# crowsonkb/style_transfer2

Measured on AMD Instinct MI355X. Metric: style-transfer iters/sec @1024px VGG19, higher is better.
Workload: dtype f32; 1 GPU; configs[1]: 1024x1024 single image per GPU, VGG19 to conv5_1, content conv4_2 + 5 style layers, adam fp32, 500 iterations per image; jobs=1, parallelism=independent jobs, 1 per GPU, no collective (replicas)

## Files before the change

style_transfer2_amd/csrc/conv3x3_winograd.hip:

```cpp
#include <hip/hip_runtime.h>
#include <stdint.h>
#include <stdlib.h>
#include <string.h>
#include <type_traits>
#include "st2_kernels.h"
#include "env.h"

namespace st2 {

typedef float f32x16 __attribute__((ext_vector_type(16)));
typedef float f32x4 __attribute__((ext_vector_type(4)));


constexpr int WN_CH = 8;
constexpr int WN_IW = 40;
constexpr int WN_V = 4 * 16 * 64;

size_t wino_pack_floats(int K, int M) { return (size_t)((M + 127) / 128 * 4) * (K / 2) * 1024; }

static void wino_pack(const float* w, int Cout, int Cin, bool dgrad, float* dst)
{
    const int K = dgrad ? Cout : Cin, M = dgrad ? Cin : Cout, nkp = K / 2;
    memset(dst, 0, wino_pack_floats(K, M) * sizeof(float));
    static const double G[4][3] = {{1, 0, 0}, {0.5, 0.5, 0.5}, {0.5, -0.5, 0.5}, {0, 0, 1}};
    for (int m = 0; m < M; ++m)
        for (int k = 0; k < K; ++k) {
            double g[3][3], t[4][3], u[4][4];
            for (int tap = 0; tap < 9; ++tap)
                g[tap / 3][tap % 3] = dgrad ? w[((size_t)k * Cin + m) * 9 + (8 - tap)] : w[((size_t)m * Cin + k) * 9 + tap];
            for (int i = 0; i < 4; ++i)
                for (int j = 0; j < 3; ++j) t[i][j] = G[i][0] * g[0][j] + G[i][1] * g[1][j] + G[i][2] * g[2][j];
            for (int i = 0; i < 4; ++i)
                for (int j = 0; j < 4; ++j) u[i][j] = t[i][0] * G[j][0] + t[i][1] * G[j][1] + t[i][2] * G[j][2];
            const size_t base = ((size_t)(m / 32) * nkp + k / 2) * 1024;
            const int lane = (k & 1) * 32 + (m & 31);
            for (int pos = 0; pos < 16; ++pos)
                dst[base + ((size_t)(pos >> 2) * 64 + lane) * 4 + (pos & 3)] = (float)u[pos >> 2][pos & 3];
        }
}
void pack_wino_weights_fwd(const float* w, int Cout, int Cin, float* dst) { wino_pack(w, Cout, Cin, false, dst); }
void pack_wino_weights_dgrad(const float* w, int Cout, int Cin, float* dst) { wino_pack(w, Cout, Cin, true, dst); }

struct WinoKArgs {
    const float* in; const float4* upack; const float* bias; float* out;
    const float* mask_src; const float* inject;
    int K, M, H, W, nch, tiles_x, tiles_y, n_mtiles, relu;
    unsigned in_bytes, u_bytes;
    float* pool_out; int pool_h, pool_w;
    unsigned char* pool_amap;
    const unsigned char* unpool_amap; unsigned amap_bytes; int ph, pw;
    int splits; float* scratch;
    unsigned long long* stamps;
};

typedef __attribute__((address_space(3))) void* lptr_t;
constexpr unsigned kOOB = 0xffffffffu;

__device__ __forceinline__ float f4c(const float4& v, int i) { return i == 0 ? v.x : i == 1 ? v.y : i == 2 ? v.z : v.w; }

template <int EPI, bool RS> struct WinoEpiOps {
    static constexpr bool E_FWD = EPI == 1 || EPI == 2, E_MASK = EPI == 3;
    static constexpr int NEB = RS ? 2 : 4;
    static constexpr int NG = E_MASK ? 2 * NEB : NEB;
    static constexpr int UNDER = NG < 4 ? NG : 4;
    int mw, dm0, odd;
    bool live, has_inj;
    unsigned row0, plane4, out_bytes;
    float mk[E_MASK ? NEB : 1][E_MASK ? 4 : 1][4], ij[E_FWD ? 1 : NEB][E_FWD ? 1 : 4][4], bs[E_FWD ? NEB : 1][E_FWD ? 4 : 1];

    __device__ __forceinline__ void init(const WinoKArgs& a, int lane, int yw, int x0, int m0, int ph, unsigned plane)
    {
        odd = lane & 1;
        const int gy = yw + 2 * ((lane & 31) >> 4) + odd;
        const int gx4 = x0 + 2 * (lane & 14);
        live = gx4 < a.W && gy < a.H;
        mw = m0 + 4 * (lane >> 5);
        dm0 = RS ? 16 * ph : 0;
        has_inj = a.inject != nullptr;
        plane4 = plane * 4u;
        out_bytes = (unsigned)a.M * plane4;
        row0 = ((unsigned)mw * plane + (live ? (unsigned)gy * a.W + gx4 : 0u)) * 4u;
    }
    __device__ __forceinline__ unsigned row_off(const WinoKArgs& a, int ebl, int ee) const
    {
        const int dm = dm0 + 8 * ebl + ee;
        return (live & (mw + dm < a.M)) ? row0 + (unsigned)dm * plane4 : kOOB;
    }
    __device__ __forceinline__ void load(const WinoKArgs& a, int g)
    {
        const int ebl = E_MASK ? g >> 1 : g;
        const bool mask = E_MASK && (g & 1) == 0;
        const __amdgpu_buffer_rsrc_t rs = E_FWD ? __builtin_amdgcn_make_buffer_rsrc((void*)a.bias, 0, (unsigned)a.M * 4u, 0x00020000)
                                        : mask ? __builtin_amdgcn_make_buffer_rsrc((void*)a.mask_src, 0, out_bytes, 0x00020000)
                                               : __builtin_amdgcn_make_buffer_rsrc((void*)a.inject, 0, has_inj ? out_bytes : 0u, 0x00020000);
#pragma unroll
        for (int ee = 0; ee < 4; ++ee) {
            if constexpr (E_FWD) {
                bs[ebl][ee] = __builtin_bit_cast(float, __builtin_amdgcn_raw_buffer_load_b32(rs, (mw + dm0 + 8 * ebl + ee) * 4, 0, 0));
            } else {
                const uint4 v = __builtin_bit_cast(uint4, __builtin_amdgcn_raw_buffer_load_b128(rs, row_off(a, ebl, ee), 0, 0));
                float (&d4)[4] = mask ? mk[E_MASK ? ebl : 0][E_MASK ? ee : 0] : ij[ebl][ee];
                d4[0] = __builtin_bit_cast(float, v.x); d4[1] = __builtin_bit_cast(float, v.y); d4[2] = __builtin_bit_cast(float, v.z); d4[3] = __builtin_bit_cast(float, v.w);
            }
        }
        asm volatile("" ::: "memory");
    }
};
template <bool RS> struct WinoEpiOps<0, RS> {};

template <int WM, int TG, int DIAG = 0, bool QUAD = true, bool PS = false, bool W8 = false, bool H4 = false, bool UNPOOL = false, bool BIG = false,
          bool NOOUT = false, int EPI = 0>
__device__ __forceinline__ void conv3x3_wino_body(const WinoKArgs& a)
{
    static_assert(EPI == 0 || (QUAD && TG == 1 && !PS && !W8 && !BIG && DIAG == 0), "specialised epilogues: aligned widths, one tile group, four waves, below 4 GiB");
    static_assert(!NOOUT || EPI == 0 || EPI == 2, "no-output builds pool");
    static_assert(!NOOUT || (QUAD && TG == 1 && !PS && !W8 && !UNPOOL && !BIG && DIAG == 0), "no-output builds: the builds that write the arg-max map");
    static_assert(!BIG || (QUAD && TG == 1 && !PS && !W8 && DIAG == 0), "big tensors: aligned widths, one tile group, four waves");
    static_assert(!UNPOOL || (QUAD && TG == 1 && !PS && !W8), "unpool: aligned widths, one tile group, four waves");
    static_assert(H4 || (WM * TG == 4 && (TG == 1 || TG == 2)), "4 waves");
    static_assert(!PS || (WM == 2 && TG == 2), "position split: 2 channel slices x 2 position halves");
    static_assert(!W8 || (WM == 4 && TG == 1 && QUAD && !PS), "eight waves: 4 channel slices x 2 position halves, aligned widths");
    static_assert(!H4 || (WM == 2 && TG == 1 && QUAD && !PS && !W8), "half tile: 2 channel slices x 2 position halves, aligned widths");
    constexpr bool RS = W8 || H4;
    constexpr bool AMAP = QUAD && TG == 1;
    constexpr int NW = W8 ? 8 : 4;
    constexpr int PARTNER = W8 ? 4 : 2;
    constexpr bool SPLIT = PS || RS;
    constexpr int BM = 32 * WM;
    constexpr int PROWS = 4 * TG;
    constexpr int IN_ROWS = PROWS + 2;
    constexpr int IW = QUAD ? WN_IW : 64;
    constexpr int COL0 = QUAD ? 3 : 0;
    constexpr int PLANE = IN_ROWS * IW;
    constexpr int UP_ROWS = PROWS / 2 + 2, UP_COLS = 24;
    constexpr int UP_PLANE = UP_ROWS * UP_COLS;
    constexpr int UP_F = WN_CH * UP_PLANE;
    constexpr int UP_FQ = UP_F / 256, UP_AQ = UP_F / 256;
    static_assert(!UNPOOL || (UP_F % 256 == 0 && NW == 4), "unpool staging is a whole number of wave-DMAs");
    constexpr int N_RAW = UNPOOL ? UP_F + UP_F / 4 : WN_CH * PLANE;
    constexpr int I_PER_WAVE = UNPOOL ? (UP_FQ + UP_AQ + NW - 1) / NW
                             : QUAD ? (N_RAW / 4 + 64 * NW - 1) / (64 * NW) : WN_CH * IN_ROWS / 4;
    constexpr int RAW = UNPOOL ? 1024 : QUAD ? I_PER_WAVE * NW * 256 : N_RAW;
    static_assert(QUAD || (WN_CH * IN_ROWS) % 4 == 0, "rows divide over the four waves");

    __shared__ __attribute__((aligned(16))) float raw_s[2][RAW];
    __shared__ __attribute__((aligned(16))) float v_s[2][TG][WN_V];
    __shared__ __attribute__((aligned(16))) float x8_own[W8 ? 8 * 8 * 64 * 4 : 4];
    static_assert(!H4 || 4 * 8 * 64 * 4 <= 2 * TG * WN_V, "H4: the exchange buffer fits the V images");
    float* const x8_s = H4 ? &v_s[0][0][0] : x8_own;

    const int tid = threadIdx.x;
    const int lane = tid & 63;
    const int wave = __builtin_amdgcn_readfirstlane(tid >> 6);
    const int wave_m = W8 ? (wave & 3) : H4 ? (wave & 1) : wave / TG, wave_g = RS ? 0 : wave % TG;
    const int ph = W8 ? wave >> 2 : H4 ? wave >> 1 : wave_g;

    const int nwg = gridDim.x / a.splits;
    const int split = blockIdx.x / nwg, orig = blockIdx.x - split * nwg;
    const int nch = a.nch / a.splits, c_first = split * nch;
    const int xcd = orig & 7, q = nwg >> 3, r = nwg & 7;
    const int logical = (xcd < r ? xcd * (q + 1) : r * (q + 1) + (xcd - r) * q) + (orig >> 3);
    const int n_pt = a.tiles_x * a.tiles_y;
    const int mt = logical / n_pt;
    const int pt = logical - mt * n_pt;
    const int tx = pt % a.tiles_x;
    const int ty = pt / a.tiles_x;
    const int y0 = ty * PROWS, x0 = tx * 32;
    const unsigned plane = (unsigned)a.H * a.W;
    const int nkp = a.K >> 1;

    const unsigned long long t_begin = DIAG ? __builtin_amdgcn_s_memtime() : 0ull;

    const __amdgpu_buffer_rsrc_t rs_i = __builtin_amdgcn_make_buffer_rsrc((void*)a.in, 0, a.in_bytes, 0x00020000);
    const __amdgpu_buffer_rsrc_t rs_a = __builtin_amdgcn_make_buffer_rsrc((void*)(UNPOOL ? a.unpool_amap : nullptr), 0, UNPOOL ? a.amap_bytes : 0u, 0x00020000);
    const unsigned pplane = UNPOOL ? (unsigned)a.ph * a.pw : 0u;
    unsigned ioff[QUAD ? I_PER_WAVE : 1];
    if (UNPOOL) {
#pragma unroll
        for (int t = 0; t < I_PER_WAVE; ++t) {
            const int piece = wave + NW * t;
            const bool bytes = piece >= UP_FQ;
            const int e = ((bytes ? piece - UP_FQ : piece) * 64 + lane) * 4;
            const int c = e / UP_PLANE;
            const int rem = e - c * UP_PLANE;
            const int rr = rem / UP_COLS;
            const int col = rem - rr * UP_COLS;
            const int gy = (y0 >> 1) - 1 + rr, gx = (x0 >> 1) - 4 + col;
            const bool ok = piece < UP_FQ + UP_AQ && gy >= 0 && gy < a.ph && gx >= 0 && gx + 3 < a.pw;
            ioff[t] = ok ? ((unsigned)((BIG && !bytes ? 0 : c_first * WN_CH) + c) * pplane + (unsigned)gy * a.pw + gx) * (bytes ? 1u : 4u) : kOOB;
        }
    } else if (QUAD) {
#pragma unroll
        for (int t = 0; t < I_PER_WAVE; ++t) {
            const int e = ((wave + NW * t) * 64 + lane) * 4;
            const int c = e / PLANE;
            const int rem = e - c * PLANE;
            const int rr = rem / IW;
            const int col = rem - rr * IW;
            const int gy = y0 - 1 + rr, gx = x0 - 4 + col;
            const bool ok = e < N_RAW && gy >= 0 && gy < a.H && gx >= 0 && gx + 3 < a.W;
            ioff[t] = ok ? ((unsigned)((BIG ? 0 : c_first * WN_CH) + c) * plane + (unsigned)gy * a.W + gx) * 4u : kOOB;
        }
    } else {
        const int gx = x0 - 1 + lane;
        ioff[0] = (lane < 34 && gx >= 0 && gx < a.W) ? (unsigned)gx * 4u : kOOB;
    }
    auto dma_raw = [&](int ch, int buf) {
        const __amdgpu_buffer_rsrc_t rs_c = BIG ? __builtin_amdgcn_make_buffer_rsrc(
            (void*)(a.in + (size_t)(c_first + ch) * WN_CH * (UNPOOL ? pplane : plane)), 0, a.in_bytes, 0x00020000) : rs_i;
        if (UNPOOL) {
#pragma unroll
            for (int t = 0; t < I_PER_WAVE; ++t) {
                const int piece = wave + NW * t;
                if (piece < UP_FQ) {
                    const unsigned vo = (ioff[t] == kOOB || BIG) ? ioff[t] : ioff[t] + (unsigned)ch * WN_CH * pplane * 4u;
                    __builtin_amdgcn_raw_ptr_buffer_load_lds(rs_c, (lptr_t)(raw_s[buf] + piece * 256), 16, vo, 0, 0, 0);
                } else if (piece < UP_FQ + UP_AQ) {
                    const unsigned vo = ioff[t] == kOOB ? kOOB : ioff[t] + (unsigned)ch * WN_CH * pplane;
                    __builtin_amdgcn_raw_ptr_buffer_load_lds(rs_a, (lptr_t)(raw_s[buf] + UP_F + (piece - UP_FQ) * 64), 4, vo, 0, 0, 0);
                }
            }
        } else if (QUAD) {
            const unsigned coff = BIG ? 0u : (unsigned)ch * WN_CH * plane * 4u;
#pragma unroll
            for (int t = 0; t < I_PER_WAVE; ++t) {
                const unsigned vo = ioff[t] == kOOB ? kOOB : ioff[t] + coff;
                __builtin_amdgcn_raw_ptr_buffer_load_lds(rs_c, (lptr_t)(raw_s[buf] + (wave + NW * t) * 256), 16, vo, 0, 0, 0);
            }
        } else {
#pragma unroll
            for (int t = 0; t < I_PER_WAVE; ++t) {
                const int row = wave + 4 * t;
                const int c = row / IN_ROWS, gy = y0 - 1 + (row - c * IN_ROWS);
                const bool row_ok = gy >= 0 && gy < a.H;
                const unsigned base = ((unsigned)((c_first + ch) * WN_CH + c) * plane + (unsigned)(row_ok ? gy : 0) * a.W) * 4u;
                const unsigned vo = (row_ok && ioff[0] != kOOB) ? ioff[0] + base : kOOB;
                __builtin_amdgcn_raw_ptr_buffer_load_lds(rs_i, (lptr_t)(raw_s[buf] + row * 64), 4, vo, 0, 0, 0);
            }
        }
    };

    const int xt = tid & 31, xch = (tid >> 5) & 7;
    const int x_raw = UNPOOL ? xch * UP_PLANE + (xt >> 4) * UP_COLS + (xt & 15) + 3
                             : xch * PLANE + (2 * (xt >> 4)) * IW + 2 * (xt & 15) + COL0;
    const int x_v = (((xch >> 1) * 4) * 64 + (xch & 1) * 32 + xt) * 4;
    float d[TG][16];
    auto pin = [&]() {
#pragma unroll
        for (int g = 0; g < TG; ++g) {
            asm volatile("" : "+v"(d[g][0]), "+v"(d[g][1]), "+v"(d[g][2]), "+v"(d[g][3]), "+v"(d[g][4]), "+v"(d[g][5]), "+v"(d[g][6]), "+v"(d[g][7]));
            asm volatile("" : "+v"(d[g][8]), "+v"(d[g][9]), "+v"(d[g][10]), "+v"(d[g][11]), "+v"(d[g][12]), "+v"(d[g][13]), "+v"(d[g][14]), "+v"(d[g][15]));
        }
    };
    float up_v[UNPOOL ? 9 : 1];
    unsigned up_m[UNPOOL ? 9 : 1];
    auto up_expand = [&]() {
        if constexpr (UNPOOL) {
#pragma unroll
            for (int i = 0; i < 4; ++i)
#pragma unroll
                for (int j = 0; j < 4; ++j) {
                    const int r = (i + 1) >> 1, cc = (j + 1) >> 1;
                    const unsigned want = 4u | (2u * ((i + 1) & 1)) | ((j + 1) & 1);
                    d[0][4 * i + j] = up_m[3 * r + cc] == want ? up_v[3 * r + cc] : 0.f;
                }
        }
    };
    auto xf_read = [&](const float* rp) {
        if constexpr (UNPOOL) {
            const unsigned char* bp = reinterpret_cast<const unsigned char*>(rp - x_raw + UP_F) + x_raw;
#pragma unroll
            for (int r = 0; r < 3; ++r)
#pragma unroll
                for (int cc = 0; cc < 3; ++cc) {
                    up_v[3 * r + cc] = rp[r * UP_COLS + cc];
                    up_m[3 * r + cc] = bp[r * UP_COLS + cc];
                }
            return;
        }
#pragma unroll
        for (int g = 0; g < TG; ++g)
#pragma unroll
            for (int i = 0; i < 4; ++i)
#pragma unroll
                for (int j = 0; j < 4; ++j) d[g][4 * i + j] = rp[(4 * g + i) * IW + j];
    };
    auto xf_math = [&]() {
#pragma unroll
        for (int g = 0; g < TG; ++g) {
            float wv[16];
#pragma unroll
            for (int j = 0; j < 4; ++j) {
                wv[j] = d[g][j] - d[g][8 + j]; wv[4 + j] = d[g][4 + j] + d[g][8 + j];
                wv[8 + j] = d[g][8 + j] - d[g][4 + j]; wv[12 + j] = d[g][4 + j] - d[g][12 + j];
            }
#pragma unroll
            for (int i = 0; i < 4; ++i) {
                d[g][4 * i] = wv[4 * i] - wv[4 * i + 2]; d[g][4 * i + 1] = wv[4 * i + 1] + wv[4 * i + 2];
                d[g][4 * i + 2] = wv[4 * i + 2] - wv[4 * i + 1]; d[g][4 * i + 3] = wv[4 * i + 1] - wv[4 * i + 3];
            }
        }
    };
    auto xf_write = [&](float* vp) {
#pragma unroll
        for (int g = 0; g < TG; ++g)
#pragma unroll
            for (int i = 0; i < 4; ++i)
                *reinterpret_cast<float4*>(vp + g * WN_V + i * 256) = make_float4(d[g][4 * i], d[g][4 * i + 1], d[g][4 * i + 2], d[g][4 * i + 3]);
    };

    const f32x4* up = reinterpret_cast<const f32x4*>(a.upack) + ((size_t)(mt * WM + wave_m) * nkp + 4 * c_first) * 256 + lane;
    constexpr int UQ = SPLIT ? 2 : 4;
    f32x4 ua[4][UQ];
    auto u_fill = [&](int kp) {
#pragma unroll
        for (int g = 0; g < UQ; ++g) ua[kp & 3][g] = up[((size_t)kp * 4 + (SPLIT ? 2 * ph + g : g)) * 64];
        asm volatile("" ::: "memory");
    };
    auto u_pin = [&](int set) {
        if constexpr (SPLIT) asm volatile("" : "+v"(ua[set][0]), "+v"(ua[set][1]));
        else asm volatile("" : "+v"(ua[set][0]), "+v"(ua[set][1]), "+v"(ua[set][2]), "+v"(ua[set][3]));
    };
    constexpr int NACC = RS ? 8 : 16;
    constexpr int NBQ = NACC / 4;
    f32x4 bq[2][NBQ];
    auto b_fetch = [&](int buf, int kpl, int set) {
#pragma unroll
        for (int pg = 0; pg < NBQ; ++pg) {
            const float* vimg = PS ? v_s[buf][pg >> 1] : v_s[buf][wave_g];
            const int quad = PS ? 2 * ph + (pg & 1) : (RS ? 2 * ph + pg : pg);
            bq[set][pg] = *reinterpret_cast<const f32x4*>(vimg + ((kpl * 4 + quad) * 64 + lane) * 4);
        }
    };
    auto b_pin = [&](int set) {
        if constexpr (RS) asm volatile("" : "+v"(bq[set][1]));
        else asm volatile("" : "+v"(bq[set][1]), "+v"(bq[set][2]), "+v"(bq[set][3]));
    };

    f32x16 acc[NACC];
#pragma unroll
    for (int p = 0; p < NACC; ++p)
#pragma unroll
        for (int e = 0; e < 16; ++e) acc[p][e] = 0.f;

    dma_raw(0, 0);
    if (nch > 1) dma_raw(1, 1);
    u_fill(0); u_fill(1); u_fill(2);
    __syncthreads();
    if (!W8 || ph == 0) {
        xf_read(raw_s[0] + x_raw);
        up_expand();
        xf_math();
        xf_write(&v_s[0][0][0] + x_v);
    }
    __syncthreads();
    b_fetch(0, 0, 0);

    unsigned long long t0 = 0, r0 = 0;
    if (DIAG) { t0 = __builtin_amdgcn_s_memtime(); r0 = __builtin_amdgcn_s_memrealtime(); }

    WinoEpiOps<EPI, RS> eo;
    if constexpr (EPI != 0) eo.init(a, lane, y0 + 4 * wave_g, x0, mt * BM + wave_m * 32, ph, plane);

    auto chunk = [&](const int c, auto more_t, auto more2_t) {
        constexpr bool MORE = decltype(more_t)::value, MORE2 = decltype(more2_t)::value;
        const int cur = c & 1;
        const bool do_xf = !W8 || ph == ((c + 1) & 1);
#pragma unroll
        for (int kpl = 0; kpl < 4; ++kpl) {
            const int kp = 4 * c + kpl;
            const int set = kpl & 1;
#pragma unroll
            for (int p = 0; p < NACC; ++p) {
                acc[p] = __builtin_amdgcn_mfma_f32_32x32x2f32(ua[kpl][SPLIT ? (p >> 2) & 1 : p >> 2][p & 3], bq[set][p >> 2][p & 3], acc[p], 0, 0, 0);
                if (p == 0) {
                    __builtin_amdgcn_sched_barrier(0);
                    b_pin(set);
                    if (kpl < 3) b_fetch(cur, kpl + 1, set ^ 1);
                    else if (MORE) {
                        if constexpr (SPLIT) asm volatile("s_waitcnt vmcnt(4) lgkmcnt(0)\n\ts_barrier" ::: "memory");
                        else asm volatile("s_waitcnt vmcnt(8) lgkmcnt(0)\n\ts_barrier" ::: "memory");
                        b_fetch(cur ^ 1, 0, 0);
                    }
                    if (MORE || kpl == 0) u_fill(kp + 3);
                    if constexpr (EPI != 0) {
                        if constexpr (!MORE) {
                            constexpr int UNDER = WinoEpiOps<EPI, RS>::UNDER;
                            if (kpl >= 4 - UNDER) eo.load(a, kpl - (4 - UNDER));
                        }
                    }
                    if (MORE && do_xf) {
                        if (kpl == 0) xf_read(raw_s[cur ^ 1] + x_raw);
                        if (kpl == 1) { up_expand(); pin(); xf_math(); pin(); }
                        if (kpl == 2) xf_write(&v_s[cur ^ 1][0][0] + x_v);
                    }
                    if (MORE2 && kpl == 0) dma_raw(c + 2, cur);
                    if (MORE || kpl < 3) u_pin((kpl + 1) & 3);
                    __builtin_amdgcn_sched_barrier(0);
                }
            }
            __builtin_amdgcn_sched_barrier(0);
        }
    };
    {
        using T = std::true_type; using F = std::false_type;
        int c = 0;
        for (; c + 2 < nch; ++c) chunk(c, T{}, T{});
        if (c + 1 < nch) { chunk(c, T{}, F{}); ++c; }
        chunk(c, F{}, F{});
    }
    if constexpr (EPI != 0) {
        if constexpr (!RS && EPI == 2) {
#pragma unroll
            for (int p = 0; p < NACC; ++p) asm volatile("" : "+a"(acc[p]));
        }
#pragma unroll
        for (int g = WinoEpiOps<EPI, RS>::UNDER; g < WinoEpiOps<EPI, RS>::NG; ++g) eo.load(a, g);
        asm volatile("" : "+v"(eo.row0));
        __builtin_amdgcn_sched_barrier(0);
    }

    unsigned long long t_loop_end = 0;
    if (DIAG) {
        const unsigned long long t1 = __builtin_amdgcn_s_memtime(), r1 = __builtin_amdgcn_s_memrealtime();
        t_loop_end = t1;
        if (tid == 0 && a.stamps) { a.stamps[2 * blockIdx.x] = t1 - t0; a.stamps[2 * blockIdx.x + 1] = r1 - r0; }
    }
    float* const xbuf = &v_s[0][0][0];
    auto partial_out = [&](auto grp_t, auto e0_t, int el, float (&y)[4]) {
        constexpr int grp = decltype(grp_t)::value, e0 = decltype(e0_t)::value;
        float t0[4], t1[4];
#pragma unroll
        for (int j = 0; j < 4; ++j) {
            const float ra = acc[(grp * 8 + j) % NACC][e0 + el], rb = acc[(grp * 8 + 4 + j) % NACC][e0 + el];
            if (ph == 0) { t0[j] = ra + rb; t1[j] = rb; }
            else { t0[j] = ra; t1[j] = -ra - rb; }
        }
        y[0] = t0[0] + t0[1] + t0[2]; y[1] = t0[1] - t0[2] - t0[3];
        y[2] = t1[0] + t1[1] + t1[2]; y[3] = t1[1] - t1[2] - t1[3];
    };
    if constexpr (PS) {
        __syncthreads();
#pragma unroll
        for (int e = 0; e < 16; ++e) {
            float y[4];
            if (wave_g == 0) partial_out(std::integral_constant<int, 1>{}, std::integral_constant<int, 0>{}, e, y);
            else partial_out(std::integral_constant<int, 0>{}, std::integral_constant<int, 0>{}, e, y);
            *reinterpret_cast<float4*>(xbuf + ((wave * 16 + e) * 64 + lane) * 4) = make_float4(y[0], y[1], y[2], y[3]);
        }
        __syncthreads();
    }
    if constexpr (RS) {
        if constexpr (H4) __syncthreads();
#pragma unroll
        for (int el = 0; el < 8; ++el) {
            float y[4];
            if (ph == 0) partial_out(std::integral_constant<int, 0>{}, std::integral_constant<int, 8>{}, el, y);
            else partial_out(std::integral_constant<int, 0>{}, std::integral_constant<int, 0>{}, el, y);
            *reinterpret_cast<float4*>(x8_s + ((wave * 8 + el) * 64 + lane) * 4) = make_float4(y[0], y[1], y[2], y[3]);
        }
        __syncthreads();
    }
    auto out_xf = [&](int e, float& y00, float& y01, float& y10, float& y11) {
        if constexpr (RS) {
            float y[4];
            if (ph == 0) partial_out(std::integral_constant<int, 0>{}, std::integral_constant<int, 0>{}, e, y);
            else partial_out(std::integral_constant<int, 0>{}, std::integral_constant<int, 8>{}, e, y);
            const float4 o = *reinterpret_cast<const float4*>(x8_s + (((wave ^ PARTNER) * 8 + e) * 64 + lane) * 4);
            y00 = y[0] + o.x; y01 = y[1] + o.y; y10 = y[2] + o.z; y11 = y[3] + o.w;
        } else if constexpr (PS) {
            float y[4];
            if (wave_g == 0) partial_out(std::integral_constant<int, 0>{}, std::integral_constant<int, 0>{}, e, y);
            else partial_out(std::integral_constant<int, 1>{}, std::integral_constant<int, 0>{}, e, y);
            const float4 o = *reinterpret_cast<const float4*>(xbuf + (((wave ^ 1) * 16 + e) * 64 + lane) * 4);
            y00 = y[0] + o.x; y01 = y[1] + o.y; y10 = y[2] + o.z; y11 = y[3] + o.w;
        } else {
            float tt[2][4];
#pragma unroll
            for (int j = 0; j < 4; ++j) {
                tt[0][j] = acc[j][e] + acc[4 + j][e] + acc[(8 + j) % NACC][e];
                tt[1][j] = acc[4 + j][e] - acc[(8 + j) % NACC][e] - acc[(12 + j) % NACC][e];
            }
            y00 = tt[0][0] + tt[0][1] + tt[0][2]; y01 = tt[0][1] - tt[0][2] - tt[0][3];
            y10 = tt[1][0] + tt[1][1] + tt[1][2]; y11 = tt[1][1] - tt[1][2] - tt[1][3];
        }
    };
  if (!QUAD) {
    const int t31 = lane & 31, khalf = lane >> 5;
    const int gy0 = y0 + 4 * wave_g + 2 * (t31 >> 4), gx = x0 + 2 * (t31 & 15);
    const bool part = a.splits > 1;
    const bool has_bias = !part && a.bias != nullptr, has_mask = !part && a.mask_src != nullptr, has_inj = !part && a.inject != nullptr;
    const bool relu = !part && a.relu;
    float* const outp = part ? a.scratch + (size_t)split * a.M * plane : a.out;
    const bool live = gx < a.W && gy0 < a.H;
    const bool row1 = gy0 + 1 < a.H, col1 = gx + 1 < a.W, wide = (a.W & 1) == 0;
    const int mw = mt * BM + wave_m * 32 + 4 * khalf;
    const unsigned pix0 = live ? (unsigned)gy0 * a.W + gx : 0u, pix1 = (live && row1) ? pix0 + a.W : pix0;
    auto ld2 = [&](const float* base, unsigned off) -> float2 {
        if (wide) return *reinterpret_cast<const float2*>(base + off);
        return make_float2(base[off], col1 ? base[off + 1] : 0.f);
    };
#pragma unroll
    for (int eb = 0; eb < 4; ++eb) {
        const int mb = mw + 8 * eb;
        unsigned off[4];
        float2 mk[4][2], ij[4][2];
        float bs[4];
#pragma unroll
        for (int ee = 0; ee < 4; ++ee) {
            const int m = mb + ee < a.M ? mb + ee : a.M - 1;
            off[ee] = (unsigned)m * plane;
            bs[ee] = has_bias ? a.bias[m] : 0.f;
        }
        if (has_mask) {
#pragma unroll
            for (int ee = 0; ee < 4; ++ee) { mk[ee][0] = ld2(a.mask_src, off[ee] + pix0); mk[ee][1] = ld2(a.mask_src, off[ee] + pix1); }
        }
        if (has_inj) {
#pragma unroll
            for (int ee = 0; ee < 4; ++ee) { ij[ee][0] = ld2(a.inject, off[ee] + pix0); ij[ee][1] = ld2(a.inject, off[ee] + pix1); }
        }
#pragma unroll
        for (int ee = 0; ee < 4; ++ee) {
            const int e = 4 * eb + ee;
            float o[2][2];
            out_xf(e, o[0][0], o[0][1], o[1][0], o[1][1]);
            if (a.pool_out && live && mb + ee < a.M) {
                float pm = o[0][0];
                if (col1) pm = pm > o[0][1] ? pm : o[0][1];
                if (row1) { pm = pm > o[1][0] ? pm : o[1][0]; if (col1) pm = pm > o[1][1] ? pm : o[1][1]; }
                pm += bs[ee];
                if (relu) pm = pm > 0.f ? pm : 0.f;
                a.pool_out[((size_t)(mb + ee) * a.pool_h + (gy0 >> 1)) * a.pool_w + (gx >> 1)] = pm;
            }
#pragma unroll
            for (int i = 0; i < 2; ++i) {
                float o0 = o[i][0] + bs[ee], o1 = o[i][1] + bs[ee];
                if (relu) { o0 = o0 > 0.f ? o0 : 0.f; o1 = o1 > 0.f ? o1 : 0.f; }
                if (has_mask) { o0 = mk[ee][i].x > 0.f ? o0 : 0.f; o1 = mk[ee][i].y > 0.f ? o1 : 0.f; }
                if (has_inj) { o0 += ij[ee][i].x; o1 += ij[ee][i].y; }
                if (live && mb + ee < a.M && (i == 0 || row1)) {
                    float* dst = outp + off[ee] + (i ? pix1 : pix0);
                    if (wide) *reinterpret_cast<float2*>(dst) = make_float2(o0, o1);
                    else { dst[0] = o0; if (col1) dst[1] = o1; }
                }
            }
        }
    }
  } else if constexpr (EPI != 0) {
    constexpr bool E_FWD = EPI == 1 || EPI == 2, E_POOL = EPI == 2, E_MASK = EPI == 3;
    constexpr int NEB = RS ? 2 : 4;
    typedef unsigned wn_u32x4 __attribute__((ext_vector_type(4)));
    const int t31 = lane & 31;
    const __amdgpu_buffer_rsrc_t rs_o = __builtin_amdgcn_make_buffer_rsrc((void*)a.out, 0, NOOUT ? 0u : eo.out_bytes, 0x00020000);
    const int ty2 = y0 + 4 * wave_g + 2 * (t31 >> 4), tx2 = x0 + 2 * (t31 & 15);
    const bool plive = E_POOL && tx2 < a.W && ty2 < a.H, prow1 = ty2 + 1 < a.H;
    const unsigned pplane = E_POOL ? (unsigned)a.pool_h * a.pool_w : 0u;
    const unsigned ppix = plive ? (unsigned)(ty2 >> 1) * a.pool_w + (tx2 >> 1) : 0u;
    const __amdgpu_buffer_rsrc_t rs_po = __builtin_amdgcn_make_buffer_rsrc((void*)a.pool_out, 0, E_POOL ? (unsigned)a.M * pplane * 4u : 0u, 0x00020000);
    const __amdgpu_buffer_rsrc_t rs_pa = __builtin_amdgcn_make_buffer_rsrc((void*)a.pool_amap, 0, (E_POOL && a.pool_amap) ? (unsigned)a.M * pplane : 0u, 0x00020000);
#pragma unroll
    for (int ebl = 0; ebl < NEB; ++ebl) {
        const int mb = eo.mw + eo.dm0 + 8 * ebl;
        if constexpr (!RS && !E_POOL) {
#pragma unroll
            for (int p = 0; p < NACC; ++p) asm volatile("" : "+a"(acc[p]));
        }
#pragma unroll
        for (int ee = 0; ee < 4; ++ee) {
            const int e = 4 * ebl + ee;
            float y00, y01, y10, y11;
            out_xf(e, y00, y01, y10, y11);
            if constexpr (E_POOL) {
                const float b = eo.bs[E_FWD ? ebl : 0][E_FWD ? ee : 0];
                float pm = y00 > y01 ? y00 : y01;
                const float p1 = y10 > y11 ? y10 : y11, pm2 = pm > p1 ? pm : p1;
                pm = prow1 ? pm2 : pm;
                const float qb = pm + b;
                const unsigned slot = y00 + b == qb ? 0u : (y01 + b == qb ? 1u : (y10 + b == qb ? 2u : 3u));
                const unsigned po = (plive && mb + ee < a.M) ? (unsigned)(mb + ee) * pplane + ppix : kOOB;
                __builtin_amdgcn_raw_buffer_store_b8((unsigned char)(slot | (qb > 0.f ? 4u : 0u)), rs_pa, po, 0, 0);
                pm += b;
                pm = pm > 0.f ? pm : 0.f;
                __builtin_amdgcn_raw_buffer_store_b32(__builtin_bit_cast(unsigned, pm), rs_po, po == kOOB ? kOOB : po * 4u, 0, 0);
            }
            if constexpr (NOOUT) continue;
            const float s0 = eo.odd ? y00 : y10, s1 = eo.odd ? y01 : y11;
            const float r0 = __builtin_bit_cast(float, __builtin_amdgcn_update_dpp(0, __builtin_bit_cast(int, s0), 0xB1, 0xf, 0xf, true));
            const float r1 = __builtin_bit_cast(float, __builtin_amdgcn_update_dpp(0, __builtin_bit_cast(int, s1), 0xB1, 0xf, 0xf, true));
            float o[4];
            o[0] = eo.odd ? r0 : y00; o[1] = eo.odd ? r1 : y01; o[2] = eo.odd ? y10 : r0; o[3] = eo.odd ? y11 : r1;
#pragma unroll
            for (int j = 0; j < 4; ++j) {
                if constexpr (E_FWD) {
                    o[j] += eo.bs[E_FWD ? ebl : 0][E_FWD ? ee : 0];
                    o[j] = o[j] > 0.f ? o[j] : 0.f;
                } else {
                    if constexpr (E_MASK) o[j] = eo.mk[E_MASK ? ebl : 0][E_MASK ? ee : 0][j] > 0.f ? o[j] : 0.f;
                    const float oi = o[j] + eo.ij[E_FWD ? 0 : ebl][E_FWD ? 0 : ee][j];
                    o[j] = eo.has_inj ? oi : o[j];
                }
            }
            wn_u32x4 ov;
#pragma unroll
            for (int j = 0; j < 4; ++j) ov[j] = __builtin_bit_cast(unsigned, o[j]);
            __builtin_amdgcn_raw_buffer_store_b128(ov, rs_o, eo.row_off(a, ebl, ee), 0, 0);
        }
        __builtin_amdgcn_sched_barrier(0);
    }
  } else {
    const int t31 = lane & 31, khalf = lane >> 5;
    const int odd = lane & 1;
    const int gy = y0 + 4 * wave_g + 2 * (t31 >> 4) + odd;
    const int gx4 = x0 + 2 * (t31 & 14);
    const bool part = a.splits > 1;
    const bool has_bias = !part && a.bias != nullptr, has_mask = !part && a.mask_src != nullptr, has_inj = !part && a.inject != nullptr;
    const bool relu = !part && a.relu;
    float* const outp = part ? a.scratch + (size_t)split * a.M * plane : a.out;
    const bool live = gx4 < a.W && gy < a.H;
// ... 292 lines not shown
```

style_transfer2_amd/csrc/gram.hip:

```cpp
#include "st2_kernels.h"
#include "env.h"
#include "wave_reduce.h"
#include <stdint.h>
#include <stdlib.h>

namespace st2 {

typedef float f32x16 __attribute__((ext_vector_type(16)));

constexpr int GKT = 32;
constexpr int GLD = GKT + 1;

GramPlan gram_plan(int C, int hw)
{
    GramPlan p;
    p.bt = C > 64 ? 128 : 64;
    const int t = (C + p.bt - 1) / p.bt;
    p.tiles = t * (t + 1) / 2;
    const int target128 = (int)env_int("ST2_GRAM_BLOCKS", 512), target64 = (int)env_int("ST2_GRAM_BLOCKS64", 1024);
    int want = p.bt == 128 ? target128 / p.tiles : (target64 + p.tiles - 1) / p.tiles;
    const int max_splits = (hw + 4 * GKT - 1) / (4 * GKT);
    if (want > max_splits) want = max_splits;
    if (want < 1) want = 1;
    int kslab = (hw + want - 1) / want;
    kslab = (kslab + GKT - 1) / GKT * GKT;
    p.kslab = kslab;
    p.splits = (hw + kslab - 1) / kslab;
    p.slab_floats = (size_t)p.splits * C * C;
    return p;
}

GramPlan gram_plan16(int C, int hw)
{
    GramPlan p = gram_plan(C, hw);
    p.kslab = (p.kslab + 63) / 64 * 64;
    p.splits = (hw + p.kslab - 1) / p.kslab;
    p.slab_floats = (size_t)p.splits * C * C;
    return p;
}

template <int BT>
__global__ __launch_bounds__(256) void gram_partial_k(const float* __restrict__ F, float* __restrict__ slabs,
                                                      int C, int hw, int tiles_1d, int kslab, GramRoi roi)
{
    constexpr int T = BT / 64;
    constexpr int ROWS_PER_T = BT / 8;
    __shared__ float As[BT * GLD];
    __shared__ float Bs[BT * GLD];

    const int tid = threadIdx.x, lane = tid & 63, wave = tid >> 6;
    const int wm = wave >> 1, wn = wave & 1;
    const int n_ut = tiles_1d * (tiles_1d + 1) / 2;
    int tile = blockIdx.x % n_ut;
    const int split = blockIdx.x / n_ut;
    int ti = 0;
    while (tile >= tiles_1d - ti) { tile -= tiles_1d - ti; ++ti; }
    const int tj = ti + tile;
    const int i0 = ti * BT, j0 = tj * BT;
    const bool diag = ti == tj;
    const int kbeg = split * kslab;
    const int kend = min(hw, kbeg + kslab);

    const int sk = tid & 31, sr = tid >> 5;
    float ra[ROWS_PER_T], rb[ROWS_PER_T];

    auto load = [&](int k0) {
        const int k = k0 + sk;
        const int ky = k / roi.rw, kx = k - ky * roi.rw;
        const size_t pix = (size_t)(roi.y0 + ky) * roi.pitch + roi.x0 + kx;
#pragma unroll
        for (int it = 0; it < ROWS_PER_T; ++it) {
            const int r = sr + it * 8;
            ra[it] = (i0 + r < C && k < kend) ? F[(size_t)(i0 + r) * roi.plane + pix] : 0.f;
            if (!diag) rb[it] = (j0 + r < C && k < kend) ? F[(size_t)(j0 + r) * roi.plane + pix] : 0.f;
        }
    };
    auto store = [&]() {
#pragma unroll
        for (int it = 0; it < ROWS_PER_T; ++it) {
            const int r = sr + it * 8;
            As[r * GLD + sk] = ra[it];
            if (!diag) Bs[r * GLD + sk] = rb[it];
        }
    };

    f32x16 acc[T][T];
#pragma unroll
    for (int i = 0; i < T; ++i)
#pragma unroll
        for (int j = 0; j < T; ++j)
#pragma unroll
            for (int e = 0; e < 16; ++e) acc[i][j][e] = 0.f;

    const float* bsrc = diag ? As : Bs;
    const int khalf = lane >> 5, l31 = lane & 31;
    const float* a_base = As + (wm * (T * 32) + l31) * GLD + khalf;
    const float* b_base = bsrc + (wn * (T * 32) + l31) * GLD + khalf;

    load(kbeg);
    for (int k0 = kbeg; k0 < kend; k0 += GKT) {
        __syncthreads();
        store();
        __syncthreads();
        if (k0 + GKT < kend) load(k0 + GKT);
#pragma unroll
        for (int ks = 0; ks < GKT / 2; ++ks) {
            float av[T], bv[T];
#pragma unroll
            for (int i = 0; i < T; ++i) av[i] = a_base[i * 32 * GLD + 2 * ks];
#pragma unroll
            for (int j = 0; j < T; ++j) bv[j] = b_base[j * 32 * GLD + 2 * ks];
#pragma unroll
            for (int i = 0; i < T; ++i)
#pragma unroll
                for (int j = 0; j < T; ++j)
                    acc[i][j] = __builtin_amdgcn_mfma_f32_32x32x2f32(av[i], bv[j], acc[i][j], 0, 0, 0);
        }
    }

    float* dst = slabs + (size_t)split * C * C;
#pragma unroll
    for (int i = 0; i < T; ++i)
#pragma unroll
        for (int j = 0; j < T; ++j) {
            const int col = j0 + wn * (T * 32) + j * 32 + l31;
#pragma unroll
            for (int e = 0; e < 16; ++e) {
                const int row = i0 + wm * (T * 32) + i * 32 + (e & 3) + 8 * (e >> 2) + 4 * khalf;
                if (row < C && col < C) dst[(size_t)row * C + col] = acc[i][j][e];
            }
        }
}

typedef __attribute__((address_space(3))) void* gram_lptr_t;
typedef float gf32x4 __attribute__((ext_vector_type(4)));

template <int BT>
__device__ __forceinline__ void gram_partial_dma_body(const float* __restrict__ F, unsigned f_bytes, float* __restrict__ slabs,
                                                      int C, int hw, int tiles_1d, int kslab)
{
    constexpr int T = BT / 64;
    constexpr int IMG = BT * 32;
    constexpr int PIECES = IMG / 256;
    constexpr int PPW = PIECES / 4;
    __shared__ __attribute__((aligned(16))) float smem[2][2][IMG];

    const int tid = threadIdx.x, lane = tid & 63;
    const int wave = __builtin_amdgcn_readfirstlane(tid >> 6);
    const int wm = wave >> 1, wn = wave & 1;
    const int n_ut = tiles_1d * (tiles_1d + 1) / 2;
    int tile = blockIdx.x % n_ut;
    const int split = blockIdx.x / n_ut;
    int ti = 0;
    while (tile >= tiles_1d - ti) { tile -= tiles_1d - ti; ++ti; }
    const int tj = ti + tile;
    const int i0 = ti * BT, j0 = tj * BT;
    const bool diag = ti == tj;
    const int kbeg = split * kslab;
    const int kend = min(hw, kbeg + kslab);
    const int nsteps = (kend - kbeg) / 32;

    const __amdgpu_buffer_rsrc_t rs = __builtin_amdgcn_make_buffer_rsrc((void*)F, 0, f_bytes, 0x00020000);
    unsigned aoff[PPW], boff[PPW];
#pragma unroll
    for (int t = 0; t < PPW; ++t) {
        const int slot = (wave + 4 * t) * 64 + lane;
        const int r = slot >> 3, q = (slot & 7) ^ ((r >> 1) & 7);
        aoff[t] = i0 + r < C ? ((unsigned)(i0 + r) * (unsigned)hw + (unsigned)kbeg + 4u * q) * 4u : 0xffffffffu;
        boff[t] = j0 + r < C ? ((unsigned)(j0 + r) * (unsigned)hw + (unsigned)kbeg + 4u * q) * 4u : 0xffffffffu;
    }
    auto dma = [&](int step, int stage) {
        const unsigned so = (unsigned)step * 128u;
#pragma unroll
        for (int t = 0; t < PPW; ++t) {
            __builtin_amdgcn_raw_ptr_buffer_load_lds(rs, (gram_lptr_t)(smem[stage][0] + (wave + 4 * t) * 256), 16,
                                                     aoff[t] == 0xffffffffu ? aoff[t] : aoff[t] + so, 0, 0, 0);
            if (!diag)
                __builtin_amdgcn_raw_ptr_buffer_load_lds(rs, (gram_lptr_t)(smem[stage][1] + (wave + 4 * t) * 256), 16,
                                                         boff[t] == 0xffffffffu ? boff[t] : boff[t] + so, 0, 0, 0);
        }
    };

    f32x16 acc[T][T];
#pragma unroll
    for (int i = 0; i < T; ++i)
#pragma unroll
        for (int j = 0; j < T; ++j)
#pragma unroll
            for (int e = 0; e < 16; ++e) acc[i][j][e] = 0.f;

    const int l31 = lane & 31;
    const bool hi = lane >= 32;
    int arow[T], brow[T];
#pragma unroll
    for (int i = 0; i < T; ++i) { arow[i] = wm * (T * 32) + i * 32 + l31; brow[i] = wn * (T * 32) + i * 32 + l31; }

    if (nsteps > 0) dma(0, 0);
    for (int st = 0; st < nsteps; ++st) {
        const int cur = st & 1;
        asm volatile("s_waitcnt vmcnt(0)" ::: "memory");
        __syncthreads();
        if (st + 1 < nsteps) dma(st + 1, cur ^ 1);
        const float* As = smem[cur][0];
        const float* Bs = diag ? smem[cur][0] : smem[cur][1];
#pragma unroll
        for (int q = 0; q < 8; ++q) {
            float a0[T], a1[T], b0[T], b1[T];
#pragma unroll
            for (int i = 0; i < T; ++i) {
                const gf32x4 v = *reinterpret_cast<const gf32x4*>(As + (arow[i] * 8 + (q ^ ((arow[i] >> 1) & 7))) * 4);
                a0[i] = hi ? v.y : v.x; a1[i] = hi ? v.w : v.z;
            }
#pragma unroll
            for (int j = 0; j < T; ++j) {
                const gf32x4 v = *reinterpret_cast<const gf32x4*>(Bs + (brow[j] * 8 + (q ^ ((brow[j] >> 1) & 7))) * 4);
                b0[j] = hi ? v.y : v.x; b1[j] = hi ? v.w : v.z;
            }
#pragma unroll
            for (int i = 0; i < T; ++i)
#pragma unroll
                for (int j = 0; j < T; ++j) {
                    acc[i][j] = __builtin_amdgcn_mfma_f32_32x32x2f32(a0[i], b0[j], acc[i][j], 0, 0, 0);
                    acc[i][j] = __builtin_amdgcn_mfma_f32_32x32x2f32(a1[i], b1[j], acc[i][j], 0, 0, 0);
                }
        }
    }

    const int khalf = lane >> 5;
    float* dst = slabs + (size_t)split * C * C;
#pragma unroll
    for (int i = 0; i < T; ++i)
#pragma unroll
        for (int j = 0; j < T; ++j) {
            const int col = j0 + wn * (T * 32) + j * 32 + l31;
#pragma unroll
            for (int e = 0; e < 16; ++e) {
                const int row = i0 + wm * (T * 32) + i * 32 + (e & 3) + 8 * (e >> 2) + 4 * khalf;
                if (row < C && col < C) dst[(size_t)row * C + col] = acc[i][j][e];
            }
        }
}

__global__ __launch_bounds__(256, 2) void gram_partial_dma_128(const float* F, unsigned f_bytes, float* slabs, int C, int hw, int tiles_1d, int kslab)
{ gram_partial_dma_body<128>(F, f_bytes, slabs, C, hw, tiles_1d, kslab); }
__global__ __launch_bounds__(256, 2) void gram_partial_dma_64(const float* F, unsigned f_bytes, float* slabs, int C, int hw, int tiles_1d, int kslab)
{ gram_partial_dma_body<64>(F, f_bytes, slabs, C, hw, tiles_1d, kslab); }

hipError_t launch_gram_partial(const float* F, float* slabs, int C, int hw, const GramPlan& pl, hipStream_t s,
                               const GramRoi* roi_in)
{
    const int t1 = (C + pl.bt - 1) / pl.bt;
    const unsigned grid = (unsigned)(pl.tiles * pl.splits);
    GramRoi roi = roi_in ? *roi_in : GramRoi{0, 0, hw, hw, (size_t)hw};
    if (!roi_in && !env_off("ST2_GRAM_DMA") && hw % 32 == 0 && pl.kslab % 32 == 0 && (reinterpret_cast<uintptr_t>(F) & 15) == 0 &&
        4ull * C * hw < 0xfffffff0ull) {
        const unsigned fb = (unsigned)(4ull * C * hw);
        if (pl.bt == 128) gram_partial_dma_128<<<grid, 256, 0, s>>>(F, fb, slabs, C, hw, t1, pl.kslab);
        else gram_partial_dma_64<<<grid, 256, 0, s>>>(F, fb, slabs, C, hw, t1, pl.kslab);
        return hipGetLastError();
    }
    if (pl.bt == 128) gram_partial_k<128><<<grid, 256, 0, s>>>(F, slabs, C, hw, t1, pl.kslab, roi);
    else gram_partial_k<64><<<grid, 256, 0, s>>>(F, slabs, C, hw, t1, pl.kslab, roi);
    return hipGetLastError();
}

__global__ __launch_bounds__(256) void gram_reduce_k(const float* __restrict__ slabs, const float* __restrict__ target,
                                                     float* __restrict__ out, float* __restrict__ partial,
                                                     int cc, int splits, float n, int C, int out_ld, int bt)
{
    __shared__ float scratch[4];
    float acc[1] = {0.f};
    for (int i = blockIdx.x * 256 + threadIdx.x; i < cc; i += gridDim.x * 256) {
        const int r = i / C, c = i - r * C;
        const int tr = r / bt, tc = c / bt;
        if (tr > tc) continue;
        float sum = 0.f;
        for (int s = 0; s < splits; ++s) sum += slabs[(size_t)s * cc + i];
        float v = sum / n;
        if (target) v -= target[i];
        out[r * out_ld + c] = v;
        acc[0] += v * v;
        if (tr < tc) { out[c * out_ld + r] = v; acc[0] += v * v; }
    }
    block_sum(acc, scratch);
    if (threadIdx.x == 0 && partial) partial[blockIdx.x] = acc[0];
}

__global__ __launch_bounds__(256) void gram_fold_k(const float* __restrict__ slabs, float* __restrict__ folded,
                                                   int cc, int splits, int per_group, int C, int bt)
{
    const int i = blockIdx.x * 256 + threadIdx.x;
    const int g = blockIdx.y;
    if (i >= cc) return;
    if ((i / C) / bt > (i % C) / bt) return;
    const int s0 = g * per_group, s1 = min(splits, s0 + per_group);
    float sum = 0.f;
    for (int s = s0; s < s1; ++s) sum += slabs[(size_t)s * cc + i];
    folded[(size_t)g * cc + i] = sum;
}

template <int GR_LANES>
__global__ __launch_bounds__(256) void gram_reduce_wide_k(const float* __restrict__ slabs, const float* __restrict__ target,
                                                          float* __restrict__ out, float* __restrict__ partial,
                                                          int cc, int splits, float n, int C, int out_ld, int bt)
{
    constexpr int GR_QUADS = 256 / GR_LANES, GR_ELEMS = 4 * GR_QUADS;
    __shared__ float4 part_s[GR_LANES][GR_QUADS];
    __shared__ float scratch[4];
    const int q = threadIdx.x % GR_QUADS, ln = threadIdx.x / GR_QUADS;
    float acc[1] = {0.f};
    for (int base = blockIdx.x * GR_ELEMS; base < cc; base += gridDim.x * GR_ELEMS) {
        const int i = base + 4 * q;
        const int r = i < cc ? i / C : 0, c = i < cc ? i - r * C : 0;
        const bool live = i < cc && r / bt <= c / bt;
        float4 sum = make_float4(0.f, 0.f, 0.f, 0.f);
        if (live)
            for (int s = ln; s < splits; s += GR_LANES) {
                const float4 v = *reinterpret_cast<const float4*>(slabs + (size_t)s * cc + i);
                sum.x += v.x; sum.y += v.y; sum.z += v.z; sum.w += v.w;
            }
        __syncthreads();
        part_s[ln][q] = sum;
        __syncthreads();
        if (ln == 0 && live) {
            float4 tot = part_s[0][q];
#pragma unroll
            for (int j = 1; j < GR_LANES; ++j) { const float4 p = part_s[j][q]; tot.x += p.x; tot.y += p.y; tot.z += p.z; tot.w += p.w; }
            float v[4] = {tot.x / n, tot.y / n, tot.z / n, tot.w / n};
            if (target) { const float4 t = *reinterpret_cast<const float4*>(target + i); v[0] -= t.x; v[1] -= t.y; v[2] -= t.z; v[3] -= t.w; }
            const bool mirror = r / bt < c / bt;
#pragma unroll
            for (int k = 0; k < 4; ++k) {
                out[r * out_ld + c + k] = v[k];
                acc[0] += v[k] * v[k];
                if (mirror) { out[(c + k) * out_ld + r] = v[k]; acc[0] += v[k] * v[k]; }
            }
        }
    }
    block_sum(acc, scratch);
    if (threadIdx.x == 0 && partial) partial[blockIdx.x] = acc[0];
}

int gram_fold_groups(const GramPlan& pl) { return pl.splits > 32 ? 32 : 0; }

hipError_t launch_gram_reduce(const float* slabs, float* folded, const float* target, float* out, int out_ld, float* partial,
                              int* n_partial, int C, double divisor, const GramPlan& pl, hipStream_t s)
{
    const int cc = C * C;
    int splits = pl.splits;
    if (splits > 32 && C % 4 == 0 && pl.bt % 4 == 0 && env_int("ST2_GRAM_REDUCE", 1) != 2) {
        const bool small = cc <= 128 * 128;
        const int grid = reduce_grid((size_t)cc, small ? 32 : 128, kMaxPartials);
        if (n_partial) *n_partial = grid;
        if (small) gram_reduce_wide_k<32><<<grid, 256, 0, s>>>(slabs, target, out, partial, cc, splits, (float)divisor, C, out_ld, pl.bt);
        else gram_reduce_wide_k<8><<<grid, 256, 0, s>>>(slabs, target, out, partial, cc, splits, (float)divisor, C, out_ld, pl.bt);
        return hipGetLastError();
    }
    const int groups = gram_fold_groups(pl);
    if (groups) {
        const int per = (pl.splits + groups - 1) / groups;
        gram_fold_k<<<dim3((cc + 255) / 256, groups), 256, 0, s>>>(slabs, folded, cc, pl.splits, per, C, pl.bt);
        slabs = folded;
        splits = (pl.splits + per - 1) / per;
    }
    const int grid = reduce_grid((size_t)cc, 256, kMaxPartials);
    if (n_partial) *n_partial = grid;
    gram_reduce_k<<<grid, 256, 0, s>>>(slabs, target, out, partial, cc, splits, (float)divisor, C, out_ld, pl.bt);
    return hipGetLastError();
}

}
```

Measured before the change: 143.1 it/s.

## Streamline gram DMA kernel LDS reads and use buffer loads for winograd weights

The gram partial kernel now precomputes swizzled LDS pointers, reads 8-byte pairs and redistributes them with permlane32_swap instead of 16-byte reads followed by lane selects. The main loop is unrolled by two so the stage index is a compile-time constant, and diagonal tiles where both waves cover the same rows reuse the A fragments for B. The DMA passes the step offset through the buffer soffset field instead of a per-load conditional add. In the winograd conv, weight fragment loads go through raw buffer loads with an immediate offset on the H4 path, which cuts address arithmetic; the gains come at the cost of more registers and more code size.

```diff
diff --git a/style_transfer2_amd/csrc/conv3x3_winograd.hip b/style_transfer2_amd/csrc/conv3x3_winograd.hip
--- a/style_transfer2_amd/csrc/conv3x3_winograd.hip
+++ b/style_transfer2_amd/csrc/conv3x3_winograd.hip
@@ -310,11 +310,17 @@
     };
 
     const f32x4* up = reinterpret_cast<const f32x4*>(a.upack) + ((size_t)(mt * WM + wave_m) * nkp + 4 * c_first) * 256 + lane;
+    const __amdgpu_buffer_rsrc_t rs_u = __builtin_amdgcn_make_buffer_rsrc(
+        (void*)(reinterpret_cast<const char*>(a.upack) + ((size_t)(mt * WM + wave_m) * nkp + 4 * c_first) * 4096), 0, H4 ? (unsigned)nch * 16384u : 0u, 0x00020000);
+    const int up_lane = lane * 16;
     constexpr int UQ = SPLIT ? 2 : 4;
     f32x4 ua[4][UQ];
     auto u_fill = [&](int kp) {
 #pragma unroll
-        for (int g = 0; g < UQ; ++g) ua[kp & 3][g] = up[((size_t)kp * 4 + (SPLIT ? 2 * ph + g : g)) * 64];
+        for (int g = 0; g < UQ; ++g) {
+            if constexpr (H4) ua[kp & 3][g] = __builtin_bit_cast(f32x4, __builtin_amdgcn_raw_buffer_load_b128(rs_u, up_lane + (2 * ph + g) * 1024, kp * 4096, 0));
+            else ua[kp & 3][g] = up[((size_t)kp * 4 + (SPLIT ? 2 * ph + g : g)) * 64];
+        }
         asm volatile("" ::: "memory");
     };
     auto u_pin = [&](int set) {
diff --git a/style_transfer2_amd/csrc/gram.hip b/style_transfer2_amd/csrc/gram.hip
--- a/style_transfer2_amd/csrc/gram.hip
+++ b/style_transfer2_amd/csrc/gram.hip
@@ -3,6 +3,7 @@
 #include "wave_reduce.h"
 #include <stdint.h>
 #include <stdlib.h>
+#include <type_traits>
 
 namespace st2 {
 
@@ -133,7 +134,8 @@
 }
 
 typedef __attribute__((address_space(3))) void* gram_lptr_t;
-typedef float gf32x4 __attribute__((ext_vector_type(4)));
+typedef float gf32x2 __attribute__((ext_vector_type(2)));
+typedef const __attribute__((address_space(3))) gf32x2* gram_rd_t;
 
 template <int BT>
 __device__ __forceinline__ void gram_partial_dma_body(const float* __restrict__ F, unsigned f_bytes, float* __restrict__ slabs,
@@ -170,14 +172,12 @@
         boff[t] = j0 + r < C ? ((unsigned)(j0 + r) * (unsigned)hw + (unsigned)kbeg + 4u * q) * 4u : 0xffffffffu;
     }
     auto dma = [&](int step, int stage) {
-        const unsigned so = (unsigned)step * 128u;
+        const int so = step * 128;
 #pragma unroll
         for (int t = 0; t < PPW; ++t) {
-            __builtin_amdgcn_raw_ptr_buffer_load_lds(rs, (gram_lptr_t)(smem[stage][0] + (wave + 4 * t) * 256), 16,
-                                                     aoff[t] == 0xffffffffu ? aoff[t] : aoff[t] + so, 0, 0, 0);
+            __builtin_amdgcn_raw_ptr_buffer_load_lds(rs, (gram_lptr_t)(smem[stage][0] + (wave + 4 * t) * 256), 16, aoff[t], so, 0, 0);
             if (!diag)
-                __builtin_amdgcn_raw_ptr_buffer_load_lds(rs, (gram_lptr_t)(smem[stage][1] + (wave + 4 * t) * 256), 16,
-                                                         boff[t] == 0xffffffffu ? boff[t] : boff[t] + so, 0, 0, 0);
+                __builtin_amdgcn_raw_ptr_buffer_load_lds(rs, (gram_lptr_t)(smem[stage][1] + (wave + 4 * t) * 256), 16, boff[t], so, 0, 0);
         }
     };
 
@@ -189,32 +189,42 @@
 #pragma unroll
             for (int e = 0; e < 16; ++e) acc[i][j][e] = 0.f;
 
-    const int l31 = lane & 31;
-    const bool hi = lane >= 32;
-    int arow[T], brow[T];
-#pragma unroll
-    for (int i = 0; i < T; ++i) { arow[i] = wm * (T * 32) + i * 32 + l31; brow[i] = wn * (T * 32) + i * 32 + l31; }
-
-    if (nsteps > 0) dma(0, 0);
-    for (int st = 0; st < nsteps; ++st) {
-        const int cur = st & 1;
+    const int l31 = lane & 31, khalf = lane >> 5;
+    const bool same = diag && wm == wn;
+    gram_rd_t ap[T][8], bp[T][8];
+#pragma unroll
+    for (int i = 0; i < T; ++i) {
+        const int ar = wm * (T * 32) + i * 32 + l31, br = wn * (T * 32) + i * 32 + l31;
+        const int abase = ar * 32 + ((ar >> 1) & 7) * 4 + khalf * 2, bbase = (diag ? 0 : IMG) + br * 32 + ((br >> 1) & 7) * 4 + khalf * 2;
+#pragma unroll
+        for (int q = 0; q < 8; ++q) {
+            ap[i][q] = (gram_rd_t)((gram_lptr_t)(&smem[0][0][0] + (abase ^ (q * 4))));
+            bp[i][q] = (gram_rd_t)((gram_lptr_t)(&smem[0][0][0] + (bbase ^ (q * 4))));
+            asm volatile("" : "+v"(ap[i][q]), "+v"(bp[i][q]));
+        }
+    }
+
+    auto step = [&](int st, auto stage_c, auto same_c) {
+        constexpr int STAGE = decltype(stage_c)::value;
+        constexpr bool SAME = decltype(same_c)::value;
         asm volatile("s_waitcnt vmcnt(0)" ::: "memory");
         __syncthreads();
-        if (st + 1 < nsteps) dma(st + 1, cur ^ 1);
-        const float* As = smem[cur][0];
-        const float* Bs = diag ? smem[cur][0] : smem[cur][1];
+        if (st + 1 < nsteps) dma(st + 1, STAGE ^ 1);
 #pragma unroll
         for (int q = 0; q < 8; ++q) {
             float a0[T], a1[T], b0[T], b1[T];
 #pragma unroll
             for (int i = 0; i < T; ++i) {
-                const gf32x4 v = *reinterpret_cast<const gf32x4*>(As + (arow[i] * 8 + (q ^ ((arow[i] >> 1) & 7))) * 4);
-                a0[i] = hi ? v.y : v.x; a1[i] = hi ? v.w : v.z;
+                const gf32x2 v = ap[i][q][STAGE * IMG];
+                const auto x = __builtin_amdgcn_permlane32_swap(__float_as_uint(v.x), __float_as_uint(v.y), false, false);
+                a0[i] = __uint_as_float(x[0]); a1[i] = __uint_as_float(x[1]);
             }
 #pragma unroll
             for (int j = 0; j < T; ++j) {
-                const gf32x4 v = *reinterpret_cast<const gf32x4*>(Bs + (brow[j] * 8 + (q ^ ((brow[j] >> 1) & 7))) * 4);
-                b0[j] = hi ? v.y : v.x; b1[j] = hi ? v.w : v.z;
+                if (SAME) { b0[j] = a0[j]; b1[j] = a1[j]; continue; }
+                const gf32x2 v = bp[j][q][STAGE * IMG];
+                const auto x = __builtin_amdgcn_permlane32_swap(__float_as_uint(v.x), __float_as_uint(v.y), false, false);
+                b0[j] = __uint_as_float(x[0]); b1[j] = __uint_as_float(x[1]);
             }
 #pragma unroll
             for (int i = 0; i < T; ++i)
@@ -224,9 +234,19 @@
                     acc[i][j] = __builtin_amdgcn_mfma_f32_32x32x2f32(a1[i], b1[j], acc[i][j], 0, 0, 0);
                 }
         }
-    }
-
-    const int khalf = lane >> 5;
+    };
+    auto steps = [&](auto same_c) {
+        int st = 0;
+        for (; st + 1 < nsteps; st += 2) {
+            step(st, std::integral_constant<int, 0>{}, same_c);
+            step(st + 1, std::integral_constant<int, 1>{}, same_c);
+        }
+        if (st < nsteps) step(st, std::integral_constant<int, 0>{}, same_c);
+    };
+    if (nsteps > 0) dma(0, 0);
+    if (same) steps(std::true_type{});
+    else steps(std::false_type{});
+
     float* dst = slabs + (size_t)split * C * C;
 #pragma unroll
     for (int i = 0; i < T; ++i)
```

Result: no change. 143.9 it/s (median of 6 runs) (+0.6%).
